# vanTeeffelenLab/ExTrack

Measured on AMD Instinct MI355X. Metric: log-likelihood evals/sec (1e6 tracks, 2-state, len=30), higher is better.
Workload: dtype f64

## Files before the change

extrack_amd/csrc/xt_reg2.h:

```cpp
#pragma once
#include "xt_fast2.h"
#include "xt_grad.h"


template <int F>
struct XtR2Geom {
    static constexpr int NGB = F - 1;
    static constexpr int NG = 1 << NGB;
    static constexpr int TPW = 64 / NG;
};
XT_HD constexpr int xt_r2_gbit(int F, int i) { return F == 7 ? i : (i < 2 ? i : i + 1); }
XT_HD constexpr int xt_r2_gmask(int F) { return F == 7 ? 63 : (F == 6 ? 0x3b : (F == 5 ? 0x1b : 0x0b)); }
template <int F>
XT_HD int xt_r2_slot(int lane)
{
    if (F == 7) return 0;
    int ts = (lane >> 2) & 1;
    if (F == 5) ts |= ((lane >> 5) & 1) << 1;
    if (F == 4) ts |= ((lane >> 4) & 3) << 1;
    return ts;
}

#define XT_R2_TAN0 XT_F2_TAB_BYTES
#define XT_R2_TB 36
// ... 95 lines not shown
    for (int d = 0; d < D; ++d) {
        dmW[d] = xt_fma(c[d], Ws, -M[d]);
        if (K == 1) dsqW = xt_fma(dmW[d], dmW[d], dsqW);
    }
    double x[2], gf[2], tt[2][K];
    const double A = -0.5 * rW * dsqW;
    XT_UNROLL
    for (int q = 0; q < 2; ++q) {
        if (K == 1) {
            x[q] = A * rD[q][0];
            tt[q][0] = xt_fma(Ws, TD2[q], U[0]) * rD[q][0];
            gf[q] = xt_pow_half<D>(Ws * rD[q][0]);
        } else {
            double xx = 0.0, gg = 1.0;
            XT_UNROLL
            for (int d = 0; d < D; ++d) {
                xx = xt_fma(dmW[d] * dmW[d], rD[q][d], xx);
                tt[q][d] = xt_fma(Ws, TD2[q], U[d]) * rD[q][d];
                gg *= Ws * rD[q][d];
            }
            x[q] = xx * (-0.5 * rW);
            gf[q] = sqrt(gg);
        }
    }
    double p[2];
    int j[2], n[2];
    xt_exp_tab_x2(x[0], x[1], p[0], p[1], j[0], j[1], n[0], n[1]);
    double nz[2], nm[2][D], nu[2][K];
    int ne[2];
    XT_UNROLL
    for (int q = 0; q < 2; ++q) {
        int en = We + n[q];
        const double tj = xt_at<double>(lds, XT_F2_EXPB_OFF + j[q] * 8);
        double zn = (Wm * TT[q]) * (gf[q] * tj) * p[q];
        if (!LAZY) {
            en += xt_frexp_exp(zn);
            zn = xt_frexp_mant(zn);
        }
        nz[q] = zn;
        ne[q] = en > XT_EMIN ? en : XT_EMIN;
        XT_UNROLL
        for (int d = 0; d < D; ++d) nm[q][d] = xt_fma(dmW[d], tt[q][K == 1 ? 0 : d], M[d]) * rW;
        XT_UNROLL
        for (int k = 0; k < K; ++k) nu[q][k] = l2[k] * tt[q][k];
    }

    double a0 = 0.0, a1 = 0.0, cm[D], cu[K], dn[D], Aq[2][K], rq[2][K];
    if (NP > 0) {
        a0 = w0 * rW;
        a1 = w1 * rW;
        const double aa = a0 * a1;
        XT_UNROLL
        for (int d = 0; d < D; ++d) {
            cm[d] = aa * (s.m[0][d] - s.m[1][d]);
            dn[d] = dmW[d] * rW;
        }
        XT_UNROLL
        for (int k = 0; k < K; ++k) cu[k] = aa * (s.u[0][k] - s.u[1][k]);
        XT_UNROLL
        for (int q = 0; q < 2; ++q)
            XT_UNROLL
            for (int k = 0; k < K; ++k) {
                rq[q][k] = Ws * rD[q][k];
                if (K == 1)
                    Aq[q][0] = -0.5 * rq[q][0] * xt_fma(-(dsqW * rW * rW), rq[q][0], (double)D);
                else
                    Aq[q][k] = -0.5 * rq[q][k] * xt_fma(-(dn[k] * dn[k]), rq[q][k], 1.0);
            }
    }
    cx.template pair_exchange<XB>(nz[0], nz[1]);
    cx.template pair_exchange_i32<XB>(ne[0], ne[1]);
    XT_UNROLL
    for (int d = 0; d < D; ++d) cx.template pair_exchange<XB>(nm[0][d], nm[1][d]);
    XT_UNROLL
    for (int k = 0; k < K; ++k) cx.template pair_exchange<XB>(nu[0][k], nu[1][k]);
    XT_UNROLL
    for (int q = 0; q < 2; ++q) {
        s.z[q] = nz[q];
        s.e[q] = ne[q];
        XT_UNROLL
        for (int d = 0; d < D; ++d) s.m[q][d] = nm[q][d];
        XT_UNROLL
        for (int k = 0; k < K; ++k) s.u[q][k] = nu[q][k];
    }
    if (NP > 0) {
        XT_UNROLL
        for (int pp = 0; pp < NP; ++pp) {
            if (!(VAR & 1)) xt_sched_fence();
            const int tb = XT_R2_TAN0 + pp * XT_R2_TB * 8;
            double dl[K];
            XT_UNROLL
            for (int k = 0; k < K; ++k) dl[k] = xt_at<double>(lds, tb + k * 8);
            const double del = s.rz[pp][0] - s.rz[pp][1];
            const double R = xt_fma(a0, s.rz[pp][0], a1 * s.rz[pp][1]);
            double dmb[D], dub[K];
            XT_UNROLL
            for (int d = 0; d < D; ++d) dmb[d] = xt_fma(cm[d], del, xt_fma(a0, s.dm[pp][0][d], a1 * s.dm[pp][1][d]));
            XT_UNROLL
            for (int k = 0; k < K; ++k) dub[k] = xt_fma(cu[k], del, xt_fma(a0, s.du[pp][0][k], a1 * s.du[pp][1][k]));
            double hd[K];
            if (K == 1) {
                hd[0] = 0.0;
                XT_UNROLL
                for (int d = 0; d < D; ++d) hd[0] = xt_fma(dn[d], dmb[d], hd[0]);
            } else {
                XT_UNROLL
                for (int d = 0; d < D; ++d) hd[d] = dn[d] * dmb[d];
            }
            double trz[2], tdm[2][D], tdu[2][K];
            XT_UNROLL
            for (int q = 0; q < 2; ++q) {
                const double dlT = xt_at<double>(lds, tb + tab + io[q]);
                const double dd2 = xt_at<double>(lds, tb + XT_R2_TAB0 + 4 * 32 + io[q]);
                double rzn = R + dlT, dtt[K];
                XT_UNROLL
                for (int k = 0; k < K; ++k) {
                    const double ds2 = dd2 + dub[k], dden = dl[k] + ds2;
                    dtt[k] = rq[q][k] * xt_fma(-tt[q][k], dden, ds2);
                    rzn = xt_fma(Aq[q][k], dden, rzn);
                    rzn = xt_fma(rq[q][k], hd[k], rzn);
                    tdu[q][k] = xt_fma(l2[k], dtt[k], dl[k] * tt[q][k]);
                }
                trz[q] = ZF ? rzn : (live ? rzn : 0.0);
                XT_UNROLL
                for (int d = 0; d < D; ++d) {
                    const int kk = K == 1 ? 0 : d;
                    tdm[q][d] = xt_fma(dn[d], dtt[kk], xt_fma(-tt[q][kk], dmb[d], dmb[d]));
                }
            }
            cx.template pair_exchange<XB>(trz[0], trz[1]);
            XT_UNROLL
            for (int d = 0; d < D; ++d) cx.template pair_exchange<XB>(tdm[0][d], tdm[1][d]);
            XT_UNROLL
            for (int k = 0; k < K; ++k) cx.template pair_exchange<XB>(tdu[0][k], tdu[1][k]);
            XT_UNROLL
            for (int q = 0; q < 2; ++q) {
                s.rz[pp][q] = trz[q];
                XT_UNROLL
                for (int d = 0; d < D; ++d) s.dm[pp][q][d] = tdm[q][d];
                XT_UNROLL
                for (int k = 0; k < K; ++k) s.du[pp][q][k] = tdu[q][k];
            }
        }
    }
}

#ifndef XT_R2_RC_H
#define XT_R2_RC_H 0
#endif
#define XT_R2_RC_NONE (-2147483647 - 1)
#ifndef XT_R2_STAGE_FAST
#define XT_R2_STAGE_FAST(D) ((D) < 3)
#endif
#ifndef XT_R2_STAGE_GRP
#define XT_R2_STAGE_GRP 4
#endif
#define XT_R2_IO_BITS 5
template <int F, int H, class Ctx>
XT_HD int xt_r2_pack_io(int lane)
{
    constexpr int NGB = F - 1;
    if constexpr (H >= NGB) {
        return 0;
    } else {
        constexpr int XB = xt_r2_gbit(F, H), PB = xt_r2_gbit(F, (H + NGB - 1) % NGB);
        const int prev = (lane >> PB) & 1;
        const int qa = Ctx::template pair_natural<XB>() ? 0 : (lane >> XB) & 1;
        return ((prev * 2 + qa) * 8) << (XT_R2_IO_BITS * H) | xt_r2_pack_io<F, H + 1, Ctx>(lane);
    }
}
XT_HD void xt_r2_opaque_inplace(int& pk)
{
#if defined(__HIP_DEVICE_COMPILE__)
    asm volatile("" : "+v"(pk));
#else
    (void)pk;
#endif
}
template <class Ctx>
XT_HD int xt_r2_tid8(Ctx& cx)
{
#if defined(__HIP_DEVICE_COMPILE__)
    int o;
    asm volatile("v_lshlrev_b32 %0, 3, %1" : "=v"(o) : "v"(cx.tid()));
    return o;
#else
    return cx.tid() * 8;
#endif
}
template <int F, int D, int H, bool FIRST = false, bool GAPS = false, class Ctx>
XT_HD void xt_r2_step_g(Ctx& cx, char* lds, XtR2Lane<D, 1, 0>& s, double (&lam)[2], int& pk, int tab, const double* dc, bool gap = false)
{
    constexpr int NGB = F - 1;
    constexpr int XB = xt_r2_gbit(F, H);
    xt_r2_opaque_inplace(pk);
    int io0 = (int)(((unsigned int)pk >> (XT_R2_IO_BITS * H)) & ((1u << XT_R2_IO_BITS) - 1u));
    xt_r2_opaque_inplace(io0);
    const int io[2] = {io0, io0 ^ 8};
    double TD2[2], LT[2];
    XT_UNROLL
    for (int q = 0; q < 2; ++q) {
        TD2[q] = xt_at<double>(lds, XT_R2_TAB0 + 4 * 32 + io[q]);
        LT[q] = xt_at<double>(lds, tab + XT_R2_LNT_REL + io[q]);
    }
    const double l2 = xt_at<double>(lds, 0), l22 = xt_at<double>(lds, XT_R2_GC_OFF + 8);

    double w0 = 1.0, w1 = 0.0, base = lam[0];
    if (!FIRST) {
        const double dl = lam[1] - lam[0];
        double p;
        int j, n;
        xt_exp_tab_half_x1(-fabs(dl), p, j, n);
        const double E = xt_ldexp(xt_at<double>(lds, XT_F2_EXPB_OFF + j * 8) * p, n);
        const bool up = dl < 0.0;
        w0 = s.z[0] * (up ? E : 1.0);
        w1 = s.z[1] * (up ? 1.0 : E);
        base = up ? lam[1] : lam[0];
    }
    const double Ws = FIRST ? 1.0 : w0 + w1;
    double ed[D], esq = 0.0;
    XT_UNROLL
    for (int d = 0; d < D; ++d) {
        ed[d] = FIRST ? s.m[0][d] : xt_fma(w1, s.m[1][d], w0 * s.m[0][d]);
        esq = xt_fma(ed[d], ed[d], esq);
    }
    const double V = FIRST ? s.u[0][0] : xt_fma(w1, s.u[1][0], w0 * s.u[0][0]);
    constexpr bool RN = !FIRST && (H % XT_F2_RENORM) == 0;
    const double Wm = FIRST ? s.z[0] : (RN ? xt_frexp_mant(Ws) : Ws);
    if (RN) base = xt_fma((double)xt_frexp_exp(Ws), -2.0 * XT_LN2, base);
    if (!FIRST && H == XT_R2_RC_H) {
        const int tid8 = xt_r2_tid8(cx);
        const int rc0 = xt_r2_rc0(D, 0, XtR2Geom<F>::TPW);
        const int cell = rc0 + (tid8 & ~(xt_r2_gmask(F) * 8));
        cx.atomic_max_i32(&xt_at<int>(lds, cell), (int)fmin(fmax(-base, -1e9), 1e9));
        cx.wave_sync();
        const int nsh = xt_at<int>(lds, cell);
        base += (double)nsh;
        xt_at<unsigned int>(lds, rc0 + XT_R2_RC_ARR + tid8) -= (unsigned int)nsh;
    }
    if (!FIRST && H == (XT_R2_RC_H + 1) % NGB) xt_at<int>(lds, xt_r2_rc0(D, 0, XtR2Geom<F>::TPW) + (xt_r2_tid8(cx) & ~(xt_r2_gmask(F) * 8))) = XT_R2_RC_NONE;

    const double Dq0 = xt_fma(Ws, TD2[0], V), Dq1 = xt_fma(Ws, TD2[1], V);
    const double R = xt_rcp3(Ws * (Dq0 * Dq1));
    const double h[2] = {R * Dq1, R * Dq0};
    const double l2W = FIRST ? l2 : l2 * Ws;
    const double WmW = FIRST ? Wm : Wm * Ws;
    double ny[2], nl[2], nr[2][D], nv[2];
    if constexpr (GAPS) {
        const double Dq[2] = {Dq0, Dq1};
        const double rW = FIRST ? 1.0 : R * (Dq0 * Dq1);
        const double esqg = gap ? 0.0 : esq;
        XT_UNROLL
        for (int q = 0; q < 2; ++q) {
            const double ko = l2W * h[q];
            const double k = gap ? rW : ko;
            const double yo = D == 2 ? WmW * ko : Wm * xt_pow_half<D>(FIRST ? ko : Ws * ko);
            ny[q] = gap ? Wm : yo;
            nl[q] = xt_fma(esqg, h[q], LT[q]) + base;
            XT_UNROLL
            for (int d = 0; d < D; ++d) nr[q][d] = xt_fma(ed[d], k, dc[d]);
            const double vo = xt_fma(-l2W, ko, l22);
            nv[q] = gap ? Dq[q] * rW : vo;
        }
    } else {
        XT_UNROLL
        for (int q = 0; q < 2; ++q) {
            const double k = l2W * h[q];
            ny[q] = D == 2 ? WmW * k : Wm * xt_pow_half<D>(FIRST ? k : Ws * k);
            nl[q] = xt_fma(esq, h[q], LT[q]) + base;
            XT_UNROLL
            for (int d = 0; d < D; ++d) nr[q][d] = xt_fma(ed[d], k, dc[d]);
            nv[q] = xt_fma(-l2W, k, l22);
        }
    }
    cx.template pair_exchange<XB>(ny[0], ny[1]);
    cx.template pair_exchange<XB>(nl[0], nl[1]);
    XT_UNROLL
    for (int d = 0; d < D; ++d) cx.template pair_exchange<XB>(nr[0][d], nr[1][d]);
    cx.template pair_exchange<XB>(nv[0], nv[1]);
    XT_UNROLL
    for (int q = 0; q < 2; ++q) {
        s.z[q] = ny[q];
        lam[q] = nl[q];
        XT_UNROLL
        for (int d = 0; d < D; ++d) s.m[q][d] = nr[q][d];
        s.u[q][0] = nv[q];
    }
}

template <int F, int D, bool GAPS = false, class Ctx, class GetPos>
XT_HD void xt_r2_chain_g(Ctx& cx, char* lds, XtR2Lane<D, 1, 0>& s, double (&lam)[2], int T, int stay_from, GetPos& getpos, unsigned int gm = 0u)
{
    constexpr int NGB = F - 1;
    const int lane = xt_opaque(cx.lane());
    const double l2 = xt_at<double>(lds, 0), l22 = xt_at<double>(lds, XT_R2_GC_OFF + 8);
    double y = s.z[0], la = lam[0], v = s.u[0][0];
    XT_UNROLL
    for (int t = 1; t < NGB; ++t) {
        if (t > T) break;
        const int prev = (lane >> xt_r2_gbit(F, t == 1 ? NGB - 1 : t - 2)) & 1;
        const int q = (lane >> xt_r2_gbit(F, t - 1)) & 1;
        const int io = (prev * 2 + q) * 8;
        const double LT = xt_at<double>(lds, XT_R2_LNT_OFF + (t >= stay_from ? 32 : 0) + io);
        const double d2 = xt_at<double>(lds, XT_R2_TAB0 + 4 * 32 + io);
        double dc[D], l2u[1];
        getpos(t, dc, l2u);
        const double rd = xt_rcp3(d2 + v);
        const double g = l2 * rd;
        double rsq = 0.0;
        XT_UNROLL
        for (int d = 0; d < D; ++d) rsq = xt_fma(s.m[0][d], s.m[0][d], rsq);
        if constexpr (GAPS) {
            const bool gap = (gm >> t) & 1u;
            y *= gap ? 1.0 : xt_pow_half<D>(g);
            la = xt_fma(gap ? 0.0 : rsq, rd, la + LT);
            v = gap ? d2 + v : xt_fma(-l2, g, l22);
            XT_UNROLL
            for (int d = 0; d < D; ++d) s.m[0][d] = xt_fma(s.m[0][d], gap ? 1.0 : g, dc[d]);
        } else {
            y *= xt_pow_half<D>(g);
            la = xt_fma(rsq, rd, la + LT);
            v = xt_fma(-l2, g, l22);
            XT_UNROLL
            for (int d = 0; d < D; ++d) s.m[0][d] = xt_fma(s.m[0][d], g, dc[d]);
        }
    }
    int dummy = 0;
    XT_UNROLL
    for (int i = 0; i < NGB - 1; ++i)
        if (i >= T) dummy |= 1 << xt_r2_gbit(F, i);
    const bool live = (lane & dummy) == 0;
    s.z[0] = live ? xt_frexp_mant(y) : 0.0;
    lam[0] = xt_fma((double)xt_frexp_exp(y), -2.0 * XT_LN2, la);
    s.u[0][0] = v;
}

template <int F, class Ctx>
XT_HD double xt_r2_gsum(Ctx& cx, double v)
{
    constexpr int NGB = F - 1;
    v += cx.template xor_f64<xt_r2_gbit(F, 0)>(v);
    v += cx.template xor_f64<xt_r2_gbit(F, 1)>(v);
    v += cx.template xor_f64<xt_r2_gbit(F, 2)>(v);
    if (NGB > 3) v += cx.template xor_f64<xt_r2_gbit(F, NGB > 3 ? 3 : 0)>(v);
    if (NGB > 4) v += cx.template xor_f64<xt_r2_gbit(F, NGB > 4 ? 4 : 0)>(v);
    if (NGB > 5) v += cx.template xor_f64<xt_r2_gbit(F, NGB > 5 ? 5 : 0)>(v);
    return v;
}
template <int F, class Ctx>
XT_HD int xt_r2_gmax(Ctx& cx, int v)
{
    constexpr int NGB = F - 1;
    auto mx = [](int a, int b) XT_INL { return a > b ? a : b; };
    v = mx(v, cx.template xor_i32<xt_r2_gbit(F, 0)>(v));
    v = mx(v, cx.template xor_i32<xt_r2_gbit(F, 1)>(v));
    v = mx(v, cx.template xor_i32<xt_r2_gbit(F, 2)>(v));
    if (NGB > 3) v = mx(v, cx.template xor_i32<xt_r2_gbit(F, NGB > 3 ? 3 : 0)>(v));
    if (NGB > 4) v = mx(v, cx.template xor_i32<xt_r2_gbit(F, NGB > 4 ? 4 : 0)>(v));
    if (NGB > 5) v = mx(v, cx.template xor_i32<xt_r2_gbit(F, NGB > 5 ? 5 : 0)>(v));
    return v;
}

template <int F, int D, int K, int NP, class Ctx, class GetPos>
XT_HD void xt_r2_chain(Ctx& cx, char* lds, XtR2Lane<D, K, NP>& s, int T, int stay_from, GetPos& getpos)
{
    constexpr int NGB = F - 1;
    const int lane = xt_opaque(cx.lane());
    double z = s.z[0];
    int e = s.e[0];
    XT_UNROLL
    for (int t = 1; t < NGB; ++t) {
        if (t > T) break;
        const int prev = (lane >> xt_r2_gbit(F, t == 1 ? NGB - 1 : t - 2)) & 1;
        const int q = (lane >> xt_r2_gbit(F, t - 1)) & 1;
        const int io = (prev * 2 + q) * 8;
        const double TT = xt_at<double>(lds, XT_R2_TAB0 + (t >= stay_from ? 32 : 0) + io);
        const double d2 = xt_at<double>(lds, XT_R2_TAB0 + 4 * 32 + io);
        double c[D], l2[K];
        getpos(t, c, l2);
        double tt[K], r[K], dm[D], x = 0.0, gf;
        XT_UNROLL
        for (int k = 0; k < K; ++k) {
            const double a = d2 + s.u[0][k];
            r[k] = NP == 0 ? xt_rcp3(l2[k] + a) : xt_rcp(l2[k] + a);
            tt[k] = a * r[k];
        }
        XT_UNROLL
        for (int d = 0; d < D; ++d) dm[d] = c[d] - s.m[0][d];
        if (K == 1) {
            XT_UNROLL
            for (int d = 0; d < D; ++d) x = xt_fma(dm[d], dm[d], x);
            x *= -0.5 * r[0];
            gf = xt_pow_half<D>(r[0]);
        } else {
            double gg = 1.0;
            XT_UNROLL
            for (int d = 0; d < D; ++d) {
                x = xt_fma(-0.5 * dm[d] * dm[d], r[d], x);
                gg *= r[d];
            }
            gf = sqrt(gg);
        }
        double p;
        int j, n;
        xt_exp_tab_x1(x, p, j, n);
        z = (z * TT) * (gf * xt_at<double>(lds, XT_F2_EXPB_OFF + j * 8)) * p;
        e += n;
        XT_UNROLL
        for (int d = 0; d < D; ++d) s.m[0][d] = xt_fma(dm[d], tt[K == 1 ? 0 : d], s.m[0][d]);
        XT_UNROLL
        for (int k = 0; k < K; ++k) s.u[0][k] = l2[k] * tt[k];
    }
    int dummy = 0;
    XT_UNROLL
    for (int i = 0; i < NGB - 1; ++i)
        if (i >= T) dummy |= 1 << xt_r2_gbit(F, i);
    const bool live = (lane & dummy) == 0;
    s.z[0] = live ? xt_frexp_mant(z) : 0.0;
    s.e[0] = live ? e + xt_frexp_exp(z) : XT_EMIN;
}

template <int F, int D, int K, int NP, int VAR = 0, bool GAPS = false, class Ctx>
XT_HD void xt_r2_body(const XtKernelArgs& a, const XtGradArgs& ga, Ctx& cx)
{
    static_assert(!GAPS || (NP == 0 && K == 1), "the gap-aware instantiation is the likelihood-only g-form path");
    int lb, nb;
    const XtBucketDesc b = xt_bind_bucket(a, cx.block(), cx.nblocks(), lb, nb);
    typedef XtR2Geom<F> Gm;
    constexpr int NGB = Gm::NGB, TPW = Gm::TPW;
    constexpr int GMASK = xt_r2_gmask(F);
    const int lane = cx.lane();
    const int wib = NP == 0 ? cx.uniform(cx.wave_in_block()) : cx.wave_in_block();
    const int nwb = cx.waves_per_block();
    const int L = b.L;
    const int KS = a.locerr_mode ? a.KS : 0;
    double* smem = cx.smem();
    char* lds = (char*)smem;

    const int ntab = xt_tab_doubles(2, 2);
    for (int i = cx.tid(); i < ntab; i += cx.nthreads()) smem[i] = xt_blob_ptr(a)[i];
    if (NP > 0)
        for (int i = cx.tid(); i < NP * XT_R2_TB; i += cx.nthreads()) xt_at<double>(lds, XT_R2_TAN0 + i * 8) = ga.dblob[i];
    const int NU = NP > 0 ? ga.NU : 0, NPT = NP + NU;
    for (int i = cx.tid(); i < NU * XT_R2_TB; i += cx.nthreads()) xt_at<double>(lds, XT_R2_TAN0 + (NP * XT_R2_TB + i) * 8) = ga.udblob[i];
    cx.sync();
    xt_f2_check_lds_base(lds);
    xt_f2_build_exp_table(cx, lds, XT_F2_EXPB_OFF, (const double*)(lds + XT_F2_T64_OFF));
    const bool gform = GAPS || (NP == 0 && K == 1 && a.well_scaled == 2 && a.locerr_mode == 0);
    if constexpr (NP == 0 && K == 1) {
        if (gform && cx.tid() < 10) {
            const int i = cx.tid();
            const double l2 = smem[0];
            if (i < 8)
                xt_at<double>(lds, XT_R2_LNT_OFF + i * 8) = -2.0 * (log(smem[XT_BLOB_HDR + i]) - 0.5 * D * log(l2));
            else
                xt_at<double>(lds, XT_R2_GC_OFF + (i - 8) * 8) = i == 8 ? (GAPS ? 0.5 * D * (XT_LOG2PI + log(l2)) : -0.5 / l2) : 2.0 * l2;
        }
    }
    cx.sync();
    const double* hdr = smem;

    const int ts = xt_r2_slot<F>(lane);
    const bool leader = (lane & GMASK) == 0;
    const int tlast = L - 1;
    const int stay_from = a.min_len > 2 ? a.min_len : 2;
    const int vfin = (b.isBL ? 2 : 0) + (tlast >= stay_from ? 1 : 0);
    double l2g[K];
    XT_UNROLL
    for (int k = 0; k < K; ++k) l2g[k] = hdr[k];
    int pk = xt_r2_pack_io<F, 0, Ctx>(lane);
    const bool well_scaled = GAPS || a.well_scaled != 0;
    const bool chain = NP == 0 && well_scaled;

    double* pos = (double*)(lds + xt_r2_pos0(NPT)) + wib * TPW * XT_F2_CHUNK * (D + KS);
    double* sig = pos + TPW * XT_F2_CHUNK * D;
    const int posb = NP == 0 ? xt_opaque(xt_r2_pos0(0) + (wib * TPW * XT_F2_CHUNK * (D + KS) + ts * XT_F2_CHUNK * D) * 8) : 0;
    double* accp = (double*)(lds + xt_r2_acc0(NPT, D, KS, TPW)) + (wib * 8 + ts) * (NPT + 3);
    auto accb = [&]() XT_INL { return xt_r2_acc0(0, D, KS, TPW) + (wib * 8 + xt_r2_slot<F>(xt_opaque(cx.lane()))) * 24; };
    auto rcacc = [&]() XT_INL { return xt_r2_rc0(D, KS, TPW) + XT_R2_RC_ARR + xt_opaque(cx.tid()) * 8; };
    auto rcsum = [&]() XT_INL { return xt_r2_rc0(D, KS, TPW) + 2 * XT_R2_RC_ARR + (wib * 8 + xt_r2_slot<F>(xt_opaque(cx.lane()))) * 8; };
    if (leader) {
        if (NP == 0) {
            const int ab = accb();
            xt_at<double>(lds, ab) = 1.0;
            xt_at<double>(lds, ab + 8) = 0.0;
            xt_at<double>(lds, ab + 16) = 0.0;
// ... 27 lines not shown
                unsigned int t_;
                bool ok, nx;
                const unsigned int off = elem(p0, ln + 64u * (k0 + g), t_, ok, nx);
                v[g] = xt_gld(base, off);
                vn[g] = xt_gld(base, off + (nx ? D * 8u : 0u));
            }
        };
        auto stage_st = [&](int p0, int k0, const double* v, const double* vn) XT_INL {
            const unsigned int posw = xt_r2_pos0(0) + wib * TPW * XT_F2_CHUNK * D * 8, ln = (unsigned int)xt_opaque(cx.lane()) & 63u;
            XT_UNROLL
            for (int g = 0; g < GRP; ++g) {
                if (k0 + g >= NIT) continue;
                const unsigned int i = ln + 64u * (k0 + g);
                unsigned int t_;
                bool ok, nx;
                elem(p0, i, t_, ok, nx);
                if (ok) {
                    xt_at<double>(lds, (int)(posw + i * 8u)) = gform ? vn[g] - v[g] : v[g];
                    if (v[g] != v[g]) xt_at<int>(lds, XT_F2_NAN_OFF + (wib * 8 + (int)t_) * 4) = 1;
                }
            }
        };
        auto stage = [&](int p0) XT_INL {
            cx.wave_sync();
            if constexpr (GAPS) {
                const int gc0 = xt_r2_gap0(D, TPW) + wib * 8 * 16;
                const unsigned int ln = (unsigned int)xt_opaque(cx.lane()) & 63u;
                if (ln < 8u) {
                    xt_at<uint32_t>(lds, gc0 + (int)ln * 16) = 0u;
                    xt_at<uint32_t>(lds, gc0 + (int)ln * 16 + 4) = 0u;
                }
                cx.wave_sync();
                const int64_t left = b.N - batch * TPW;
                const unsigned int tmax = left < TPW ? (unsigned int)left - 1u : (unsigned int)TPW - 1u;
                const double* const base = b.tracks + xt_uniform64(cx, batch * TPW * L * D);
                auto gelem = [&](unsigned int i, unsigned int& t_, unsigned int& row, unsigned int& pp, unsigned int& o0) XT_INL {
                    t_ = i / (XT_F2_CHUNK * D);
                    const unsigned int r = i - t_ * (XT_F2_CHUNK * D);
                    row = r / D;
                    pp = (unsigned int)p0 + row;
                    const unsigned int tc = t_ < tmax ? t_ : tmax;
                    o0 = (tc * (unsigned int)L * D + (r - row * D)) * 8u;
                    return (NE % 64 == 0 || i < NE) && pp < (unsigned int)L;
                };
                double v[NIT], vn[NIT];
                XT_UNROLL
                for (int k = 0; k < NIT; ++k) {
                    unsigned int t_, row, pp, o0;
                    const bool ok = gelem(ln + 64u * k, t_, row, pp, o0);
                    const unsigned int off = ok ? o0 + pp * (D * 8u) : 0u;
                    v[k] = xt_gld(base, off);
                    vn[k] = xt_gld(base, off + (ok && pp + 1 < (unsigned int)L ? D * 8u : 0u));
                }
                XT_UNROLL
                for (int k = 0; k < NIT; ++k) {
                    unsigned int t_, row, pp, o0;
                    if (gelem(ln + 64u * k, t_, row, pp, o0)) cx.atomic_or_u32(&xt_at<uint32_t>(lds, gc0 + (int)t_ * 16 + (v[k] != v[k] ? 0 : 4)), 1u << row);
                }
                cx.wave_sync();
                XT_UNROLL
                for (int k = 0; k < NIT; ++k) {
                    const unsigned int i = ln + 64u * k;
                    unsigned int t_, row, pp, o0;
                    if (!gelem(i, t_, row, pp, o0)) continue;
                    const unsigned int gmm = xt_at<uint32_t>(lds, gc0 + (int)t_ * 16) & ~xt_at<uint32_t>(lds, gc0 + (int)t_ * 16 + 4);
                    const bool isgap = (gmm >> row) & 1u;
                    double cur = v[k];
                    if (isgap) {
                        const unsigned int x = ~gmm & (0xffffffffu >> (31u - row));
                        const unsigned int src = x ? (unsigned int)p0 + 31u - (unsigned int)__builtin_clz(x) : (unsigned int)xt_at<int>(lds, gc0 + (int)t_ * 16 + 8);
                        cur = xt_gld(base, o0 + src * (D * 8u));
                    }
                    xt_at<double>(lds, xt_r2_pos0(0) + (wib * TPW * XT_F2_CHUNK * D + (int)i) * 8) = vn[k] != vn[k] ? 0.0 : vn[k] - cur;
                    if ((v[k] != v[k] && !isgap) || (isgap && (pp == 0u || pp + 1u == (unsigned int)L))) xt_at<int>(lds, XT_F2_NAN_OFF + (wib * 8 + (int)t_) * 4) = 1;
                }
                cx.wave_sync();
                if (ln < (unsigned int)TPW) {
                    const int cell = gc0 + (int)ln * 16;
                    const int nrows = L - p0 < XT_F2_CHUNK ? L - p0 : XT_F2_CHUNK;
                    const unsigned int valid = 0xffffffffu >> (32 - nrows);
                    const unsigned int gmm = xt_at<uint32_t>(lds, cell) & ~xt_at<uint32_t>(lds, cell + 4) & valid, obs = ~gmm & valid;
                    xt_at<uint32_t>(lds, cell) = gmm;
                    if (obs) xt_at<int>(lds, cell + 8) = p0 + 31 - __builtin_clz(obs);
                    xt_at<int>(lds, cell + 12) += __builtin_popcount(gmm);
                }
                cx.wave_sync();
                return;
            }
            if constexpr (FAST) {
                if (KS == 0 && (batch + 1) * TPW <= b.N) {
                    XT_UNROLL
                    for (int k0 = 0; k0 < NIT; k0 += GRP) {
                        double v[GRP], vn[GRP];
                        stage_ld(batch, p0, k0, v, vn);
                        stage_st(p0, k0, v, vn);
                    }
                    cx.wave_sync();
                    return;
                }
            }
            for (int i = lane; i < TPW * XT_F2_CHUNK * D; i += 64) {
                const int t_ = i / (XT_F2_CHUNK * D), r = i - t_ * (XT_F2_CHUNK * D);
                const int64_t tk = batch * TPW + t_;
                const int64_t tkc = tk < b.N ? tk : b.N - 1;
                const int pp = p0 + r / D;
                if (pp < L) {
                    const double* const src = b.tracks + (tkc * L + p0) * D + r;
                    const double v = src[0];
                    if constexpr (NP == 0 && K == 1) {
                        const double vn = src[pp + 1 < L ? D : 0];
                        pos[i] = gform ? vn - v : v;
                    } else {
                        pos[i] = v;
                    }
                    if (v != v) xt_at<int>(lds, XT_F2_NAN_OFF + (wib * 8 + t_) * 4) = 1;
                }
            }
            if (KS)
                for (int i = lane; i < TPW * XT_F2_CHUNK * KS; i += 64) {
                    const int t_ = i / (XT_F2_CHUNK * KS), r = i - t_ * (XT_F2_CHUNK * KS);
                    const int64_t tk = batch * TPW + t_;
                    const int64_t tkc = tk < b.N ? tk : b.N - 1;
                    const int pp = p0 + r / KS;
                    if (pp < L) {
                        const double v = b.sigma[(tkc * L + p0) * KS + r];
                        sig[i] = v;
                        if (v != v) xt_at<int>(lds, XT_F2_NAN_OFF + (wib * 8 + t_) * 4) = 1;
                    }
                }
            cx.wave_sync();
        };
        auto getpos = [&](int t, double* c, double* l2) XT_INL {
            const int r = t & (XT_F2_CHUNK - 1);
            XT_UNROLL
            for (int d = 0; d < D; ++d) c[d] = NP == 0 ? xt_at<double>(lds, posb + (r * D + d) * 8) : pos[(ts * XT_F2_CHUNK + r) * D + d];
            if (KS == 0) {
                XT_UNROLL
                for (int k = 0; k < K; ++k) l2[k] = xt_at<double>(lds, k * 8);
            } else {
                XT_UNROLL
                for (int k = 0; k < K; ++k) {
                    double sg = sig[(ts * XT_F2_CHUNK + r) * KS + (KS == 1 ? 0 : k)];
                    if (a.locerr_mode == 2) {
                        sg = xt_fma(sg, hdr[3], hdr[4]);
                        sg = sg < 1e-6 ? 1e-6 : sg;
                    }
                    l2[k] = sg * sg;
                }
            }
        };

        XtR2Lane<D, K, NP> s;
        double lam[2] = {0.0, 0.0};
        unsigned int gmk = 0u;
#define XT_R2_PHASE(H, ZF_, LAZY_)                                                                     \
    if (NGB > (H) && t <= tend2 && ph == (H)) {                                                        \
        double c[D], l2[K];                                                                            \
        getpos(t, c, l2);                                                                              \
        xt_r2_step<F, D, K, NP, ((H) < NGB ? (H) : 0), ZF_, LAZY_, VAR>(cx, lds, s, XT_R2_TABSEL, c, l2);   \
        ++t;                                                                                           \
        ph = (H) + 1 == NGB ? 0 : (H) + 1;                                                             \
    }
#define XT_R2_PHASE_G(H)                                                                               \
    if (NGB > (H) && t <= tend2 && ph == (H)) {                                                        \
        double c[D], l2[K];                                                                            \
        getpos(t, c, l2);                                                                              \
        xt_r2_step_g<F, D, ((H) < NGB ? (H) : 0), false, GAPS>(cx, lds, s, lam, pk, XT_R2_TABSEL, c, GAPS && ((gmk >> (t & (XT_F2_CHUNK - 1))) & 1u)); \
        ++t;                                                                                           \
        ph = (H) + 1 == NGB ? 0 : (H) + 1;                                                             \
    }
#define XT_R2_PHASES(ZF_, LAZY_) \
    XT_R2_PHASE(0, ZF_, LAZY_)   \
    XT_R2_PHASE(1, ZF_, LAZY_)   \
    XT_R2_PHASE(2, ZF_, LAZY_)   \
    XT_R2_PHASE(3, ZF_, LAZY_)   \
    XT_R2_PHASE(4, ZF_, LAZY_)   \
    XT_R2_PHASE(5, ZF_, LAZY_)
#define XT_R2_TABSEL tab
        auto run_steps = [&](int& t, int tend, int tab) XT_INL {
            int ph = (t - 1) % NGB;
            const int tend2 = tend;
            if (!well_scaled) {
                while (t <= tend2) { XT_R2_PHASES(false, false) }
                return;
            }
            if constexpr (NP == 0 && K == 1) {
                if (gform) {
                    while (t <= tend2) {
                        XT_R2_PHASE_G(0)
                        XT_R2_PHASE_G(1)
                        XT_R2_PHASE_G(2)
                        XT_R2_PHASE_G(3)
                        XT_R2_PHASE_G(4)
                        XT_R2_PHASE_G(5)
                    }
                    return;
                }
            }
            while (t <= tend2) { XT_R2_PHASES(true, true) }
        };
#undef XT_R2_TABSEL
#define XT_R2_TABSEL (XT_R2_TAB0 + (t >= stay_from ? 32 : 0))
        auto run_steps_g = [&](int& t, int tend) XT_INL {
            int ph = (t - 1) % NGB;
            const int tend2 = tend;
            if (well_scaled) {
                while (t <= tend2) { XT_R2_PHASES(false, true) }
            } else {
                while (t <= tend2) { XT_R2_PHASES(false, false) }
            }
        };
#undef XT_R2_TABSEL
#undef XT_R2_PHASES
#undef XT_R2_PHASE_G
#undef XT_R2_PHASE

        XtAcc tot;
        tot.clear();
        double gacc[NP ? NP : 1];
        double uacc[XT_R2_MAXU];
        int fe = XT_EMIN;
        int t = 1;
        if (lane < 8) xt_at<int>(lds, XT_F2_NAN_OFF + (wib * 8 + lane) * 4) = 0;
        if constexpr (GAPS) {
            if (lane < 8) {
                xt_at<int>(lds, xt_r2_gap0(D, TPW) + (wib * 8 + lane) * 16 + 8) = 0;
                xt_at<int>(lds, xt_r2_gap0(D, TPW) + (wib * 8 + lane) * 16 + 12) = 0;
            }
        }
        if (NP == 0) {
            xt_at<int>(lds, rcacc()) = 0;
            xt_at<int>(lds, rcacc() - XT_R2_RC_ARR) = XT_R2_RC_NONE;
        }
        for (int p0 = 0; p0 < L; p0 += XT_F2_CHUNK) {
            stage(p0);
            if constexpr (GAPS) gmk = xt_at<uint32_t>(lds, xt_r2_gap0(D, TPW) + (wib * 8 + xt_r2_slot<F>(xt_opaque(cx.lane()))) * 16);
            if (p0 == 0) {
                constexpr int NBIT = xt_r2_gbit(F, NGB - 1);
                double c0[D], l20[K];
                getpos(0, c0, l20);
                const bool live0 = chain || (lane & (GMASK & ~(1 << NBIT))) == 0;
                const int s0 = (lane >> NBIT) & 1;
                s.z[0] = live0 ? hdr[8 + s0] : 0.0;
                s.e[0] = live0 ? 0 : XT_EMIN;
                s.z[1] = 0.0;
                s.e[1] = XT_EMIN;
                XT_UNROLL
                for (int q = 0; q < 2; ++q) {
                    XT_UNROLL
                    for (int d = 0; d < D; ++d) s.m[q][d] = c0[d];
                    XT_UNROLL
                    for (int k = 0; k < K; ++k) s.u[q][k] = l20[k];
                }
                if constexpr (NP == 0 && K == 1) {
                    if (gform) s.u[0][0] = s.u[1][0] = 2.0 * l20[0];
                }
                XT_UNROLL
                for (int pp = 0; pp < NP; ++pp) {
                    const int tb = XT_R2_TAN0 + pp * XT_R2_TB * 8;
                    s.rz[pp][0] = live0 ? xt_at<double>(lds, tb + (8 + s0) * 8) : 0.0;
                    s.rz[pp][1] = 0.0;
                    XT_UNROLL
                    for (int q = 0; q < 2; ++q) {
                        XT_UNROLL
                        for (int d = 0; d < D; ++d) s.dm[pp][q][d] = 0.0;
                        XT_UNROLL
                        for (int k = 0; k < K; ++k) s.du[pp][q][k] = xt_at<double>(lds, tb + k * 8);
                    }
                }
                if constexpr (NP == 0) {
                    if (chain) {
                        const int T = L - 2 < NGB - 1 ? L - 2 : NGB - 1;
                        bool chain_done = false;
                        if constexpr (K == 1) {
                            if (gform) {
                                xt_r2_chain_g<F, D, GAPS>(cx, lds, s, lam, T, stay_from, getpos, gmk);
                                s.e[0] = s.e[1] = 0;
                                chain_done = true;
                            }
                        }
                        if (!chain_done) xt_r2_chain<F>(cx, lds, s, T, stay_from, getpos);
                        if (L - 2 >= F - 1) {
                            double c[D], l2[K];
                            getpos(F - 1, c, l2);
                            bool first_done = false;
                            if constexpr (K == 1) {
                                if (gform) {
                                    xt_r2_step_g<F, D, NGB - 1, true, GAPS>(cx, lds, s, lam, pk, XT_R2_TAB0 + (F - 1 >= stay_from ? 32 : 0), c, GAPS && ((gmk >> (F - 1)) & 1u));
                                    first_done = true;
                                }
                            }
                            if (!first_done) xt_r2_step<F, D, K, NP, NGB - 1, true, true, VAR, true>(cx, lds, s, XT_R2_TAB0 + (F - 1 >= stay_from ? 32 : 0), c, l2);
                            t = F;
                        } else {
                            t = L - 1 > 1 ? L - 1 : 1;
                        }
                    }
                }
            }
            const int tend = (L - 2 < p0 + XT_F2_CHUNK - 1) ? L - 2 : p0 + XT_F2_CHUNK - 1;
            if (NP == 0) {
                run_steps(t, tend < stay_from - 1 ? tend : stay_from - 1, XT_R2_TAB0);
                run_steps(t, tend, XT_R2_TAB0 + 32);
            } else {
                run_steps_g(t, tend);
            }
            if (tlast < p0 || tlast >= p0 + XT_F2_CHUNK) continue;
            double cl[D], l2l[K];
            getpos(tlast, cl, l2l);
            if constexpr (NP == 0 && K == 1) {
                if (gform) l2l[0] = 0.0;
            }
            const int hp = (tlast - 2 + NGB) % NGB;
            const int pbit = (F == 7 || hp < 2) ? hp : hp + 1;
            const int prev = (lane >> pbit) & 1;
            double wm[4], rr[4][K], dq[2][D], dsqQ[2];
            int we[4];
            if constexpr (NP == 0 && K == 1) {
                double dn[4];
                XT_UNROLL
                for (int i = 0; i < 4; ++i) dn[i] = xt_at<double>(lds, XT_R2_TAB0 + 4 * 32 + (prev * 2 + (i & 1)) * 8) + s.u[i >> 1][0] + l2l[0];
                const double p01 = dn[0] * dn[1], p23 = dn[2] * dn[3];
                const double R = xt_rcp3(p01 * p23);
                const double r01 = R * p23, r23 = R * p01;
                rr[0][0] = r01 * dn[1];
                rr[1][0] = r01 * dn[0];
                rr[2][0] = r23 * dn[3];
                rr[3][0] = r23 * dn[2];
            }
            XT_UNROLL
            for (int Q = 0; Q < 2; ++Q) {
                dsqQ[Q] = 0.0;
                XT_UNROLL
                for (int d = 0; d < D; ++d) {
                    dq[Q][d] = cl[d] - s.m[Q][d];
                    if constexpr (NP == 0 && K == 1) {
                        if (gform) dq[Q][d] = s.m[Q][d];
                    }
                    dsqQ[Q] = xt_fma(dq[Q][d], dq[Q][d], dsqQ[Q]);
                }
                double x[2], gf[2];
                XT_UNROLL
                for (int q = 0; q < 2; ++q) {
                    const double d2 = xt_at<double>(lds, XT_R2_TAB0 + 4 * 32 + (prev * 2 + q) * 8);
                    if (K == 1) {
                        double r;
                        if constexpr (NP == 0) {
                            r = rr[Q * 2 + q][0];
                        } else {
                            r = xt_rcp(d2 + s.u[Q][0] + l2l[0]);
                            rr[Q * 2 + q][0] = r;
                        }
                        if constexpr (NP == 0)
                            x[q] = -0.5 * xt_fma(dsqQ[Q], r, lam[Q]);
                        else
                            x[q] = -0.5 * dsqQ[Q] * r;
                        gf[q] = xt_pow_half<D>(r);
                    } else {
                        double xx = 0.0, gg = 1.0;
                        XT_UNROLL
                        for (int d = 0; d < D; ++d) {
                            const double r = NP == 0 ? xt_rcp3(d2 + s.u[Q][d] + l2l[d]) : xt_rcp(d2 + s.u[Q][d] + l2l[d]);
                            rr[Q * 2 + q][d] = r;
                            xx = xt_fma(-0.5 * dq[Q][d] * dq[Q][d], r, xx);
                            gg *= r;
                        }
                        x[q] = xx;
                        gf[q] = sqrt(gg);
                    }
                }
                double p[2];
                int j[2], n[2];
                xt_exp_tab_x2(x[0], x[1], p[0], p[1], j[0], j[1], n[0], n[1]);
                XT_UNROLL
                for (int q = 0; q < 2; ++q) {
                    const double tf = xt_at<double>(lds, XT_R2_TAB0 + vfin * 32 + (prev * 2 + q) * 8);
                    wm[Q * 2 + q] = s.z[Q] * tf * gf[q] * xt_at<double>(lds, XT_F2_EXPB_OFF + j[q] * 8) * p[q];
                    we[Q * 2 + q] = s.e[Q] + n[q];
                    tot.add(wm[Q * 2 + q], we[Q * 2 + q]);
                }
            }
            fe = xt_r2_gmax<F>(cx, tot.m != 0.0 ? tot.e : XT_EMIN);
            if (NP > 0) {
                double ws[4];
                XT_UNROLL
                for (int i = 0; i < 4; ++i) ws[i] = wm[i] != 0.0 ? xt_ldexp(wm[i], we[i] - fe) : 0.0;
                XT_UNROLL
                for (int pp = 0; pp < NP; ++pp) {
                    const int tb = XT_R2_TAN0 + pp * XT_R2_TB * 8;
                    double dl[K];
                    XT_UNROLL
                    for (int k = 0; k < K; ++k) dl[k] = xt_at<double>(lds, tb + k * 8);
                    double acc = 0.0;
                    XT_UNROLL
                    for (int Q = 0; Q < 2; ++Q) {
                        XT_UNROLL
                        for (int q = 0; q < 2; ++q) {
                            const double dlT = xt_at<double>(lds, tb + XT_R2_TAB0 + vfin * 32 + (prev * 2 + q) * 8);
                            const double dd2 = xt_at<double>(lds, tb + XT_R2_TAB0 + 4 * 32 + (prev * 2 + q) * 8);
                            double rel = s.rz[pp][Q] + dlT;
                            if (K == 1) {
                                const double r = rr[Q * 2 + q][0];
                                const double dden = dd2 + s.du[pp][Q][0] + dl[0];
                                double ddsq = 0.0;
                                XT_UNROLL
                                for (int d = 0; d < D; ++d) ddsq = xt_fma(-2.0 * dq[Q][d], s.dm[pp][Q][d], ddsq);
                                rel -= 0.5 * r * (D * dden + ddsq - dsqQ[Q] * r * dden);
                            } else {
                                XT_UNROLL
                                for (int d = 0; d < D; ++d) {
                                    const double r = rr[Q * 2 + q][d];
                                    const double dden = dd2 + s.du[pp][Q][d] + dl[d];
                                    rel -= 0.5 * r * (dden - 2.0 * dq[Q][d] * s.dm[pp][Q][d] - dq[Q][d] * dq[Q][d] * r * dden);
                                }
                            }
                            acc = xt_fma(ws[Q * 2 + q], ws[Q * 2 + q] != 0.0 ? rel : 0.0, acc);
                        }
                    }
                    gacc[pp] = acc;
                }
                XT_UNROLL
                for (int u = 0; u < XT_R2_MAXU; ++u) {
                    double acc = 0.0;
                    if (u < NU) {
                        const int tb = XT_R2_TAN0 + (NP + u) * XT_R2_TB * 8;
                        XT_UNROLL
                        for (int i = 0; i < 4; ++i) acc = xt_fma(ws[i], xt_at<double>(lds, tb + XT_R2_TAB0 + vfin * 32 + (prev * 2 + (i & 1)) * 8), acc);
                    }
                    uacc[u] = acc;
                }
            }
        }
        double sum = xt_r2_gsum<F>(cx, tot.m != 0.0 ? xt_ldexp(tot.m, tot.e - fe) : 0.0);
        const bool poisoned = xt_at<int>(lds, XT_F2_NAN_OFF + (wib * 8 + ts) * 4) != 0;
        if (poisoned) sum = NAN;
        if (NP == 0) {
            const int lz = xt_opaque(cx.lane());
            const int64_t trk = batch * TPW + xt_r2_slot<F>(lz);
            if (trk < b.N && (lz & GMASK) == 0) {
                double rcs = -0.5 * (double)xt_at<int>(lds, rcacc());
                if constexpr (GAPS) rcs = xt_fma((double)xt_at<int>(lds, xt_r2_gap0(D, TPW) + (wib * 8 + xt_r2_slot<F>(lz)) * 16 + 12), xt_at<double>(lds, XT_R2_GC_OFF), rcs);
                if (b.ll_out) b.ll_out[trk] = log(sum) + (double)fe * XT_LN2 + b.ll_const + rcs;
                xt_at<double>(lds, rcsum()) += rcs;
                const int ab = accb();
                const double pm = xt_at<double>(lds, ab) * xt_frexp_mant(sum);
                double acce = xt_at<double>(lds, ab + 8) + (double)(fe + xt_frexp_exp(sum) + xt_frexp_exp(pm));
                if (sum == 0.0) acce = -INFINITY;
                xt_at<double>(lds, ab) = xt_frexp_mant(pm);
                xt_at<double>(lds, ab + 8) = acce;
                xt_at<double>(lds, ab + 16) += 1.0;
            }
        } else {
            const double rs = 1.0 / sum;
            double gsum[NP ? NP : 1];
            XT_UNROLL
            for (int pp = 0; pp < NP; ++pp) gsum[pp] = xt_r2_gsum<F>(cx, gacc[pp]);
            double usum[XT_R2_MAXU];
            XT_UNROLL
            for (int u = 0; u < XT_R2_MAXU; ++u) usum[u] = u < NU ? xt_r2_gsum<F>(cx, uacc[u]) : 0.0;
            if (act && leader) {
                const double ll = log(sum) + (double)fe * XT_LN2 + b.ll_const;
                if (b.ll_out) b.ll_out[trk] = ll;
                accp[0] += ll;
                XT_UNROLL
                for (int pp = 0; pp < NP; ++pp) accp[1 + pp] += gsum[pp] * rs;
                double* const srow = b.scores_out ? b.scores_out + trk * ga.score_ld : nullptr;
                if (srow) {
                    XT_UNROLL
                    for (int pp = 0; pp < NP; ++pp) srow[ga.score_col0 + pp] = gsum[pp] * rs;
                }
                const int nsteps = L - 2 > 0 ? L - 2 : 0;
                const int n1 = nsteps >= stay_from ? nsteps - stay_from + 1 : 0, n0 = nsteps - n1;
                XT_UNROLL
                for (int u = 0; u < XT_R2_MAXU; ++u)
                    if (u < NU) {
                        const int tb = XT_R2_TAN0 + (NP + u) * XT_R2_TB * 8;
                        const double rzu = xt_at<double>(lds, tb + 8 * 8) + n0 * xt_at<double>(lds, tb + XT_R2_TAB0) + n1 * xt_at<double>(lds, tb + XT_R2_TAB0 + 32);
                        accp[1 + NP + u] += usum[u] * rs + rzu;
                        if (srow) srow[ga.score_ucol0 + u] = usum[u] * rs + rzu;
                    }
            }
        }
        cx.wave_sync();
    }

    cx.sync();
    if (NP == 0) {
        if (leader) {
            const double* ac = &xt_at<double>(lds, accb());
            smem[wib * TPW + ts] = ac[2] > 0.0 ? log(ac[0]) + ac[1] * XT_LN2 + ac[2] * b.ll_const + xt_at<double>(lds, rcsum()) : 0.0;
        }
        cx.sync();
        if (cx.tid() == 0) {
            double sacc = 0.0;
            for (int i = 0; i < nwb * TPW; ++i) sacc += smem[i];
            a.partials[cx.block()] = sacc;
        }
    } else {
        const double* acc0 = (const double*)(lds + xt_r2_acc0(NPT, D, KS, TPW));
        for (int col = cx.tid(); col < NPT + 1; col += cx.nthreads()) {
            double sacc = 0.0;
            for (int w = 0; w < nwb; ++w)
                for (int i = 0; i < TPW; ++i) sacc += acc0[(w * 8 + i) * (NPT + 3) + col];
            ga.gpartials[(int64_t)cx.block() * (NPT + 1) + col] = sacc;
        }
    }
}
```

Measured before the change: 469.8.

## Specialize gform final readout into log-domain exp evaluation with group max shift

Adds a dedicated readout path for the gform (NP==0, K==1) case. It computes per-lane log-weights, finds the group maximum with an LDS atomic max, and evaluates the final sum through the exp table with a shared integer shift. Dead lanes get NaN lambdas, and the old readout is moved into a lambda used only for the other cases. The aim is to replace the generic readout with a cheaper specialized one, at the cost of extra wave syncs and atomics, and it changes the numerics of how the shift is folded into the result.

Result: faster. 476.8 (median of 6 runs) (+1.5%).

```diff
diff --git a/extrack_amd/csrc/xt_reg2.h b/extrack_amd/csrc/xt_reg2.h
--- a/extrack_amd/csrc/xt_reg2.h
+++ b/extrack_amd/csrc/xt_reg2.h
@@ -271,6 +271,7 @@
 #ifndef XT_R2_STAGE_FAST
 #define XT_R2_STAGE_FAST(D) ((D) < 3)
 #endif
+#define XT_R2_LAM_DEAD NAN
 #ifndef XT_R2_STAGE_GRP
 #define XT_R2_STAGE_GRP 4
 #endif
@@ -450,7 +451,8 @@
         if (i >= T) dummy |= 1 << xt_r2_gbit(F, i);
     const bool live = (lane & dummy) == 0;
     s.z[0] = live ? xt_frexp_mant(y) : 0.0;
-    lam[0] = xt_fma((double)xt_frexp_exp(y), -2.0 * XT_LN2, la);
+    const double lae = xt_fma((double)xt_frexp_exp(y), -2.0 * XT_LN2, la);
+    lam[0] = live ? lae : XT_R2_LAM_DEAD;
     s.u[0][0] = v;
 }
 
@@ -784,6 +786,9 @@
 
         XtR2Lane<D, K, NP> s;
         double lam[2] = {0.0, 0.0};
+        if constexpr (NP == 0 && K == 1) {
+            if (gform) lam[1] = XT_R2_LAM_DEAD;
+        }
         unsigned int gmk = 0u;
 #define XT_R2_PHASE(H, ZF_, LAZY_)                                                                     \
     if (NGB > (H) && t <= tend2 && ph == (H)) {                                                        \
@@ -864,85 +869,9 @@
             xt_at<int>(lds, rcacc()) = 0;
             xt_at<int>(lds, rcacc() - XT_R2_RC_ARR) = XT_R2_RC_NONE;
         }
-        for (int p0 = 0; p0 < L; p0 += XT_F2_CHUNK) {
-            stage(p0);
-            if constexpr (GAPS) gmk = xt_at<uint32_t>(lds, xt_r2_gap0(D, TPW) + (wib * 8 + xt_r2_slot<F>(xt_opaque(cx.lane()))) * 16);
-            if (p0 == 0) {
-                constexpr int NBIT = xt_r2_gbit(F, NGB - 1);
-                double c0[D], l20[K];
-                getpos(0, c0, l20);
-                const bool live0 = chain || (lane & (GMASK & ~(1 << NBIT))) == 0;
-                const int s0 = (lane >> NBIT) & 1;
-                s.z[0] = live0 ? hdr[8 + s0] : 0.0;
-                s.e[0] = live0 ? 0 : XT_EMIN;
-                s.z[1] = 0.0;
-                s.e[1] = XT_EMIN;
-                XT_UNROLL
-                for (int q = 0; q < 2; ++q) {
-                    XT_UNROLL
-                    for (int d = 0; d < D; ++d) s.m[q][d] = c0[d];
-                    XT_UNROLL
-                    for (int k = 0; k < K; ++k) s.u[q][k] = l20[k];
-                }
-                if constexpr (NP == 0 && K == 1) {
-                    if (gform) s.u[0][0] = s.u[1][0] = 2.0 * l20[0];
-                }
-                XT_UNROLL
-                for (int pp = 0; pp < NP; ++pp) {
-                    const int tb = XT_R2_TAN0 + pp * XT_R2_TB * 8;
-                    s.rz[pp][0] = live0 ? xt_at<double>(lds, tb + (8 + s0) * 8) : 0.0;
-                    s.rz[pp][1] = 0.0;
-                    XT_UNROLL
-                    for (int q = 0; q < 2; ++q) {
-                        XT_UNROLL
-                        for (int d = 0; d < D; ++d) s.dm[pp][q][d] = 0.0;
-                        XT_UNROLL
-                        for (int k = 0; k < K; ++k) s.du[pp][q][k] = xt_at<double>(lds, tb + k * 8);
-                    }
-                }
-                if constexpr (NP == 0) {
-                    if (chain) {
-                        const int T = L - 2 < NGB - 1 ? L - 2 : NGB - 1;
-                        bool chain_done = false;
-                        if constexpr (K == 1) {
-                            if (gform) {
-                                xt_r2_chain_g<F, D, GAPS>(cx, lds, s, lam, T, stay_from, getpos, gmk);
-                                s.e[0] = s.e[1] = 0;
-                                chain_done = true;
-                            }
-                        }
-                        if (!chain_done) xt_r2_chain<F>(cx, lds, s, T, stay_from, getpos);
-                        if (L - 2 >= F - 1) {
-                            double c[D], l2[K];
-                            getpos(F - 1, c, l2);
-                            bool first_done = false;
-                            if constexpr (K == 1) {
-                                if (gform) {
-                                    xt_r2_step_g<F, D, NGB - 1, true, GAPS>(cx, lds, s, lam, pk, XT_R2_TAB0 + (F - 1 >= stay_from ? 32 : 0), c, GAPS && ((gmk >> (F - 1)) & 1u));
-                                    first_done = true;
-                                }
-                            }
-                            if (!first_done) xt_r2_step<F, D, K, NP, NGB - 1, true, true, VAR, true>(cx, lds, s, XT_R2_TAB0 + (F - 1 >= stay_from ? 32 : 0), c, l2);
-                            t = F;
-                        } else {
-                            t = L - 1 > 1 ? L - 1 : 1;
-                        }
-                    }
-                }
-            }
-            const int tend = (L - 2 < p0 + XT_F2_CHUNK - 1) ? L - 2 : p0 + XT_F2_CHUNK - 1;
-            if (NP == 0) {
-                run_steps(t, tend < stay_from - 1 ? tend : stay_from - 1, XT_R2_TAB0);
-                run_steps(t, tend, XT_R2_TAB0 + 32);
-            } else {
-                run_steps_g(t, tend);
-            }
-            if (tlast < p0 || tlast >= p0 + XT_F2_CHUNK) continue;
+        auto readout = [&]() XT_INL {
             double cl[D], l2l[K];
             getpos(tlast, cl, l2l);
-            if constexpr (NP == 0 && K == 1) {
-                if (gform) l2l[0] = 0.0;
-            }
             const int hp = (tlast - 2 + NGB) % NGB;
             const int pbit = (F == 7 || hp < 2) ? hp : hp + 1;
             const int prev = (lane >> pbit) & 1;
@@ -966,9 +895,6 @@
                 XT_UNROLL
                 for (int d = 0; d < D; ++d) {
                     dq[Q][d] = cl[d] - s.m[Q][d];
-                    if constexpr (NP == 0 && K == 1) {
-                        if (gform) dq[Q][d] = s.m[Q][d];
-                    }
                     dsqQ[Q] = xt_fma(dq[Q][d], dq[Q][d], dsqQ[Q]);
                 }
                 double x[2], gf[2];
@@ -1062,15 +988,153 @@
                     uacc[u] = acc;
                 }
             }
-        }
-        double sum = xt_r2_gsum<F>(cx, tot.m != 0.0 ? xt_ldexp(tot.m, tot.e - fe) : 0.0);
+        };
+        for (int p0 = 0; p0 < L; p0 += XT_F2_CHUNK) {
+            stage(p0);
+            if constexpr (GAPS) gmk = xt_at<uint32_t>(lds, xt_r2_gap0(D, TPW) + (wib * 8 + xt_r2_slot<F>(xt_opaque(cx.lane()))) * 16);
+            if (p0 == 0) {
+                constexpr int NBIT = xt_r2_gbit(F, NGB - 1);
+                double c0[D], l20[K];
+                getpos(0, c0, l20);
+                const bool live0 = chain || (lane & (GMASK & ~(1 << NBIT))) == 0;
+                const int s0 = (lane >> NBIT) & 1;
+                s.z[0] = live0 ? hdr[8 + s0] : 0.0;
+                s.e[0] = live0 ? 0 : XT_EMIN;
+                s.z[1] = 0.0;
+                s.e[1] = XT_EMIN;
+                XT_UNROLL
+                for (int q = 0; q < 2; ++q) {
+                    XT_UNROLL
+                    for (int d = 0; d < D; ++d) s.m[q][d] = c0[d];
+                    XT_UNROLL
+                    for (int k = 0; k < K; ++k) s.u[q][k] = l20[k];
+                }
+                if constexpr (NP == 0 && K == 1) {
+                    if (gform) s.u[0][0] = s.u[1][0] = 2.0 * l20[0];
+                }
+                XT_UNROLL
+                for (int pp = 0; pp < NP; ++pp) {
+                    const int tb = XT_R2_TAN0 + pp * XT_R2_TB * 8;
+                    s.rz[pp][0] = live0 ? xt_at<double>(lds, tb + (8 + s0) * 8) : 0.0;
+                    s.rz[pp][1] = 0.0;
+                    XT_UNROLL
+                    for (int q = 0; q < 2; ++q) {
+                        XT_UNROLL
+                        for (int d = 0; d < D; ++d) s.dm[pp][q][d] = 0.0;
+                        XT_UNROLL
+                        for (int k = 0; k < K; ++k) s.du[pp][q][k] = xt_at<double>(lds, tb + k * 8);
+                    }
+                }
+                if constexpr (NP == 0) {
+                    if (chain) {
+                        const int T = L - 2 < NGB - 1 ? L - 2 : NGB - 1;
+                        bool chain_done = false;
+                        if constexpr (K == 1) {
+                            if (gform) {
+                                xt_r2_chain_g<F, D, GAPS>(cx, lds, s, lam, T, stay_from, getpos, gmk);
+                                s.e[0] = s.e[1] = 0;
+                                chain_done = true;
+                            }
+                        }
+                        if (!chain_done) xt_r2_chain<F>(cx, lds, s, T, stay_from, getpos);
+                        if (L - 2 >= F - 1) {
+                            double c[D], l2[K];
+                            getpos(F - 1, c, l2);
+                            bool first_done = false;
+                            if constexpr (K == 1) {
+                                if (gform) {
+                                    xt_r2_step_g<F, D, NGB - 1, true, GAPS>(cx, lds, s, lam, pk, XT_R2_TAB0 + (F - 1 >= stay_from ? 32 : 0), c, GAPS && ((gmk >> (F - 1)) & 1u));
+                                    first_done = true;
+                                }
+                            }
+                            if (!first_done) xt_r2_step<F, D, K, NP, NGB - 1, true, true, VAR, true>(cx, lds, s, XT_R2_TAB0 + (F - 1 >= stay_from ? 32 : 0), c, l2);
+                            t = F;
+                        } else {
+                            t = L - 1 > 1 ? L - 1 : 1;
+                        }
+                    }
+                }
+            }
+            const int tend = (L - 2 < p0 + XT_F2_CHUNK - 1) ? L - 2 : p0 + XT_F2_CHUNK - 1;
+            if (NP == 0) {
+                run_steps(t, tend < stay_from - 1 ? tend : stay_from - 1, XT_R2_TAB0);
+                run_steps(t, tend, XT_R2_TAB0 + 32);
+            } else {
+                run_steps_g(t, tend);
+            }
+            if constexpr (!(NP == 0 && K == 1)) {
+                if (tlast >= p0 && tlast < p0 + XT_F2_CHUNK) readout();
+            }
+        }
+        double lsum = 0.0;
+        int ronsh = 0;
+        bool ro_log = false;
+        if constexpr (NP == 0 && K == 1) {
+            if (gform) {
+                ro_log = true;
+                const int hpl = (tlast - 2 + NGB) % NGB;
+                const int pbl = (F == 7 || hpl < 2) ? hpl : hpl + 1;
+                const int iol = ((xt_opaque(cx.lane()) >> pbl) & 1) * 16;
+                double d2l[2], tfl[2], dn[4], rho[4], aq[4], wq[4];
+                XT_UNROLL
+                for (int q = 0; q < 2; ++q) {
+                    d2l[q] = xt_at<double>(lds, XT_R2_TAB0 + 4 * 32 + iol + q * 8);
+                    tfl[q] = xt_at<double>(lds, XT_R2_TAB0 + vfin * 32 + iol + q * 8);
+                }
+                XT_UNROLL
+                for (int i = 0; i < 4; ++i) dn[i] = d2l[i & 1] + s.u[i >> 1][0];
+                const double p01 = dn[0] * dn[1], p23 = dn[2] * dn[3];
+                const double R = xt_rcp3(p01 * p23);
+                const double r01 = R * p23, r23 = R * p01;
+                rho[0] = r01 * dn[1];
+                rho[1] = r01 * dn[0];
+                rho[2] = r23 * dn[3];
+                rho[3] = r23 * dn[2];
+                XT_UNROLL
+                for (int Q = 0; Q < 2; ++Q) {
+                    double rsq = 0.0;
+                    XT_UNROLL
+                    for (int d = 0; d < D; ++d) rsq = xt_fma(s.m[Q][d], s.m[Q][d], rsq);
+                    aq[Q * 2] = xt_fma(rsq, rho[Q * 2], lam[Q]);
+                    aq[Q * 2 + 1] = xt_fma(rsq, rho[Q * 2 + 1], lam[Q]);
+                    wq[Q * 2] = (s.z[Q] * tfl[0]) * xt_pow_half<D>(rho[Q * 2]);
+                    wq[Q * 2 + 1] = (s.z[Q] * tfl[1]) * xt_pow_half<D>(rho[Q * 2 + 1]);
+                }
+                const double amin = fmin(fmin(aq[0], aq[1]), fmin(aq[2], aq[3]));
+                const int cell = xt_r2_rc0(D, 0, TPW) + (xt_r2_tid8(cx) & ~(GMASK * 8));
+                xt_at<int>(lds, cell) = XT_R2_RC_NONE;
+                cx.wave_sync();
+                cx.atomic_max_i32(&xt_at<int>(lds, cell), (int)fmin(fmax(-amin, -1e9), 1e9));
+                cx.wave_sync();
+                const int nsh = xt_at<int>(lds, cell);
+                const double nsd = -(double)nsh;
+                double acc = 0.0;
+                XT_UNROLL
+                for (int i = 0; i < 4; ++i) {
+                    double p;
+                    int j, n;
+                    xt_exp_tab_half_x1(nsd - aq[i], p, j, n);
+                    const double E = xt_ldexp(xt_at<double>(lds, XT_F2_EXPB_OFF + j * 8) * p, n);
+                    acc = xt_fma(wq[i], E, acc);
+                }
+                lsum = acc;
+                ronsh = nsh;
+                fe = 0;
+            }
+        }
+        if (!ro_log) {
+            if constexpr (NP == 0 && K == 1) readout();
+            lsum = tot.m != 0.0 ? xt_ldexp(tot.m, tot.e - fe) : 0.0;
+        }
+        double sum = xt_r2_gsum<F>(cx, lsum);
         const bool poisoned = xt_at<int>(lds, XT_F2_NAN_OFF + (wib * 8 + ts) * 4) != 0;
         if (poisoned) sum = NAN;
         if (NP == 0) {
             const int lz = xt_opaque(cx.lane());
             const int64_t trk = batch * TPW + xt_r2_slot<F>(lz);
             if (trk < b.N && (lz & GMASK) == 0) {
-                double rcs = -0.5 * (double)xt_at<int>(lds, rcacc());
+                const double rcs0 = 0.5 * ((double)ronsh - (double)xt_at<int>(lds, rcacc()));
+                double rcs = rcs0;
                 if constexpr (GAPS) rcs = xt_fma((double)xt_at<int>(lds, xt_r2_gap0(D, TPW) + (wib * 8 + xt_r2_slot<F>(lz)) * 16 + 12), xt_at<double>(lds, XT_R2_GC_OFF), rcs);
                 if (b.ll_out) b.ll_out[trk] = log(sum) + (double)fe * XT_LN2 + b.ll_const + rcs;
                 xt_at<double>(lds, rcsum()) += rcs;
```
